# edlanglois/relearn

Measured on AMD Instinct MI355X. Metric: env-steps/sec (whole node), 64k-env CartPole TRPO, higher is better.
Workload: dtype f32; 1 GPU; CartPole(VisibleStepLimit 500) MLP-TRPO, 65536 envs total, T=128, policy 5-128-2, critic 5-128-1, CG 10, <=15 backtracks, 80 Adam critic steps per period; n_envs_total=65536, n_envs_per_gpu=65536, horizon=128, hidden=128, critic_steps=80, update_chains=policy and critic chains side by side on two streams, pipeline=none, parallelism=env-sharded x1 + no collective (one rank)

## Files before the change

### relearn_amd/csrc/abi_internal.hpp

```cpp
#pragma once
#include <cmath>
#include <cstdlib>
#include <cstring>
#include <memory>
#include <string>
#include <vector>

#include "../../include/rl_chacha.h"
#include "../../include/rl_detmath.h"
#include "engine.hpp"
#include "host/cbor.hpp"
#include "kernels.hpp"

extern thread_local std::string g_last_error_no_engine;

static inline void engine_settle(rl_engine *e) {
  if (e->pending.active && !e->pending.joined) {
    RL_HIP_CHECK(hipStreamWaitEvent(e->main_stream, e->ev_join, 0));
    e->pending.joined = true;
  }
}

template <typename F>
static inline int32_t guarded(rl_engine *eng, F &&f, bool settle = true) {
// ... 59 lines not shown
                    "rl_engine_set_kernel_variant(engine, 1) for these magnitudes (include/relearn_hip.h)");
}
static inline void range_discard(rl_traj *t) {
  try {
    range_check(t);
  } catch (const RlError &) {
  }
}

enum PassKind { RUN_INIT = PASS_INIT, RUN_EVAL = PASS_EVAL, RUN_JVP = PASS_JVP, RUN_DQN = PASS_DQN, RUN_PPO = PASS_PPO,
                RUN_CRITIC, RUN_KINDS };
struct SlabRows {
  uint32_t A, B;
};
struct PassRequest {
  PassRequest(PassKind k) : kind(k) {}
  PassKind kind;
  const float *tangent = nullptr;
  const int32_t *skip = nullptr;
  float clip_lo = 0.0f, clip_hi = 0.0f;
  bool forward_only = false;
  bool reduce = true;
  uint64_t B_total = 0;
};
SlabRows run_pass(const rl_mlp *mod, rl_traj *traj, const PassRequest &req);

extern "C" {
void engine_release_child(rl_engine *e);
void traj_plan(rl_traj *t, uint64_t B);
rl_traj *traj_alloc(rl_engine *e, uint64_t n_lanes, uint64_t horizon, uint32_t obs_dim, bool resizable);
void seq_ensure(rl_traj *t, const rl_mlp *mod, bool training);
void traj_ensure_pvec(rl_traj *t, uint64_t P);
rl_mlp *seq_exec(const rl_mlp *m);
}

struct SeqScope {
  rl_traj *t;
  uint32_t logical_D;
  rl_mlp *x;
  SeqScope(rl_traj *traj, const rl_mlp *m) : t(traj), logical_D(traj->d.D), x(nullptr) {
    RL_REQUIRE(m->in_dim == traj->d.D, "module input width does not match the trajectory");
    x = seq_exec(m);
    if (!m->lane_kernels()) t->d.D = 5;
  }
  ~SeqScope() { t->d.D = logical_D; }
  SeqScope(const SeqScope &) = delete;
// ... 3 lines not shown
```

### relearn_amd/csrc/abi_update.hip

```cpp
#include "abi_internal.hpp"

enum FusedLauncher { FUSED_NONE, FUSED_POLICY ,
                     FUSED_CRITIC  };
struct PassRow {
  bool backward, sums;
  FusedLauncher fused;
};
static const PassRow PASS_TABLE[RUN_KINDS] = {
     {true, true, FUSED_POLICY},
     {false, true, FUSED_POLICY},
     {true, false, FUSED_POLICY},
     {true, true, FUSED_NONE},
     {true, true, FUSED_POLICY},
     {true, true, FUSED_CRITIC},
};
static_assert(RUN_INIT == 0 && RUN_EVAL == 1 && RUN_JVP == 2 && RUN_DQN == 3 && RUN_PPO == 4 && RUN_CRITIC == 5 &&
                  RUN_KINDS == 6,
              "PASS_TABLE rows are in the order of PassKind");

static void seq_gradient_to_flat_order(const rl_mlp *mod, rl_traj *traj) {
  if (mod->exec == nullptr) return;
  launch_seq_unpad(mod, traj->vec, mod->x_tmp);
  RL_HIP_CHECK(hipMemcpyAsync(traj->vec, mod->x_tmp, mod->P * sizeof(float), hipMemcpyDeviceToDevice, traj->eng->stream));
}
// ... 20 lines not shown
      const float *tangent = req.tangent;
      if (mod->exec != nullptr) {
        launch_seq_pad(mod, mod->x_tan, req.tangent);
        tangent = mod->x_tan;
      }
      launch_gru_tangent(traj, sc.x, tangent, Bt, req.skip);
    } else {
      launch_gru_seq_forward(traj, sc.x, traj->seq.out, nullptr, row.backward ? seq_record(traj, sc.x) : nullptr,
                             req.skip);
      if (critic) launch_seq_critic_dvalues(traj, Bt);
      else launch_seq_policy_dlogits(traj, req.kind, Bt, req.clip_lo, req.clip_hi, req.skip);
    }
    if (grad) {
      launch_gru_backward(traj, sc.x, req.skip);
      seq_gradient_to_flat_order(mod, traj);
    }
    if (row.sums) launch_reduce(traj, P, false, true, 0, traj->nbB);
    allreduce();
    return SlabRows{0, traj->nbB};
  }
  bool fused = false;
  if (traj->eng->kernel_variant == 0) {
    if (row.fused == FUSED_POLICY)
      fused = launch_policy_v2(traj, mod, req.kind, req.tangent, Bt, req.skip, req.clip_lo, req.clip_hi);
    else if (row.fused == FUSED_CRITIC)
      fused = launch_critic_step_v2(traj, mod, Bt);
  }
  if (!fused) {
    if (critic) launch_critic_fwd(traj, mod, Bt);
    else launch_policy_pass(traj, mod, req.kind, req.tangent, Bt, req.skip, req.clip_lo, req.clip_hi);
    if (row.backward) launch_mlp_backward(traj, mod, req.skip);
  }
  const SlabRows rows = fused ? SlabRows{traj->last_rows, traj->last_rows} : SlabRows{traj->nbA, traj->nbB};
  if (req.reduce) {
    launch_reduce(traj, P, row.backward, row.sums, rows.A, rows.B);
    allreduce();
  }
  return rows;
}

extern "C" {

int32_t rl_trpo_config_default(rl_trpo_config *c) {
  return guarded(nullptr, [&] {
    RL_REQUIRE(c, "cfg is NULL");
    c->iterations = 10;
    c->max_backtracks = 15;
// ... 12 lines not shown
             "policy outputs do not match the action count of the env this trajectory was collected on");
  RL_REQUIRE(policy->out_dim > traj->max_action, "the trajectory holds an action index the policy has no output for");
  if (policy->out_dim > 2 && policy->kind != RL_MODULE_MLP)
    throw RlError(RL_ERR_UNSUPPORTED, "recurrent chains are built for two actions");
}

static inline void trpo_candidate(rl_mlp *policy, rl_traj *traj, const rl_trpo_config *cfg, uint64_t i, double ratio) {
  launch_ls_set_params(traj, policy, ratio);
  PassRequest eval(RUN_EVAL);
  eval.skip = &traj->trpo->ls_accepted;
  run_pass(policy, traj, eval);
  launch_ls_check(traj, (uint32_t)policy->P, b_total(traj), (int)i, ratio, cfg->max_policy_step_kl);
}

struct TrpoProgress {
  uint64_t next = 0;
  double ratio = 1.0;
};

static TrpoProgress trpo_update_head(rl_mlp *policy, rl_traj *traj, const rl_trpo_config *cfg) {
  uint32_t P = (uint32_t)policy->P;
  uint64_t Bt = b_total(traj);
  float reg = (float)cfg->hpv_reg_coeff;
  run_pass(policy, traj, RUN_INIT);
  launch_trpo_begin(traj, policy, Bt);
  PassRequest fvp(RUN_JVP);
  fvp.tangent = traj->cg_p;
  fvp.skip = &traj->trpo->cg_done;
  for (uint64_t it = 0; it < cfg->iterations; ++it) {
    run_pass(policy, traj, fvp);
    launch_cg_step(traj, P, reg, 1e-10f);
  }
  launch_cg_finish(traj, P);
  fvp.tangent = traj->cg_x;
  fvp.skip = nullptr;
  run_pass(policy, traj, fvp);
  launch_step_size(traj, policy, reg, cfg->max_policy_step_kl);
  TrpoProgress pr;
  for (; pr.next < cfg->max_backtracks && pr.next < 2; ++pr.next) {
    if (pr.next > 0) pr.ratio *= cfg->backtrack_ratio;
    trpo_candidate(policy, traj, cfg, pr.next, pr.ratio);
  }
  return pr;
}

static void trpo_update_tail(rl_mlp *policy, rl_traj *traj, const rl_trpo_config *cfg, TrpoProgress pr,
                             rl_trpo_stats *stats) {
// ... 44 lines not shown
}

int32_t rl_policy_gradient(rl_mlp *policy, rl_traj *traj, float *grad_out, float *loss_out, float *entropy_out) {
  return guarded(traj ? traj->eng : nullptr, [&] {
    check_policy(policy, traj);
    RL_REQUIRE(grad_out, "grad_out is NULL");
    uint32_t P = (uint32_t)policy->P;
    run_pass(policy, traj, RUN_INIT);
    std::vector<float> h(P + 4);
    d2h(traj->eng, h.data(), traj->vec, (P + 4) * sizeof(float));
    range_check(traj, 1u << RL_GUARD_POLICY);
    std::memcpy(grad_out, h.data(), P * sizeof(float));
    double inv_B = 1.0 / (double)b_total(traj);
    if (loss_out) *loss_out = (float)(-((double)h[P] * inv_B));
    if (entropy_out) *entropy_out = (float)((double)h[P + 1] * inv_B);
  });
}

int32_t rl_policy_fvp(rl_mlp *policy, rl_traj *traj, const float *v, float reg, float *out) {
  return guarded(traj ? traj->eng : nullptr, [&] {
    check_policy(policy, traj);
    RL_REQUIRE(v && out, "NULL argument");
    uint32_t P = (uint32_t)policy->P;
    run_pass(policy, traj, RUN_INIT);
    h2d(traj->eng, traj->cg_x, v, P * sizeof(float));
    PassRequest fvp(RUN_JVP);
    fvp.tangent = traj->cg_x;
    run_pass(policy, traj, fvp);
    std::vector<float> h(P);
    d2h(traj->eng, h.data(), traj->vec, P * sizeof(float));
    range_check(traj, 1u << RL_GUARD_POLICY);
    for (uint32_t i = 0; i < P; ++i) out[i] = h[i] + reg * v[i];
  });
}

int32_t rl_policy_loss_kl(rl_mlp *policy, rl_traj *traj, const float *params0, float *loss_out, float *kl_out) {
  return guarded(traj ? traj->eng : nullptr, [&] {
    check_policy(policy, traj);
    RL_REQUIRE(params0 && loss_out && kl_out, "NULL argument");
    rl_engine *e = traj->eng;
    uint32_t P = (uint32_t)policy->P;
    uint64_t Bt = b_total(traj);
    std::vector<float> cur(P);
    d2h(e, cur.data(), policy->d_params, P * sizeof(float));
    h2d(e, policy->d_params, params0, P * sizeof(float));
    wimg_invalidate(policy);
    run_pass(policy, traj, RUN_INIT);
// ... 521 lines not shown
```

### relearn_amd/csrc/bf16_tile.hpp

```cpp
#pragma once
#include <hip/hip_runtime.h>

#include <cstdint>
#include <type_traits>

#include "../../include/rl_detmath.h"

namespace bt {

typedef float f32x16 __attribute__((ext_vector_type(16)));
typedef float f32x2 __attribute__((ext_vector_type(2)));
typedef __bf16 bf16x8 __attribute__((ext_vector_type(8)));
typedef __bf16 bf16x2 __attribute__((ext_vector_type(2)));

constexpr int NT = 4;
constexpr int PAR_D = 5, PAR_H = 128;
constexpr uint32_t PAR_B1 = PAR_H * PAR_D, PAR_W2 = PAR_B1 + PAR_H;
__host__ __device__ constexpr uint32_t par_b2(int A) { return PAR_W2 + (uint32_t)(A * PAR_H); }
constexpr uint32_t SHARE_OLD = 5, SHARE_YOUNG = 3;

__device__ __forceinline__ void wave_lds_fence() {
  __builtin_amdgcn_fence(__ATOMIC_RELEASE, "wavefront");
  __builtin_amdgcn_wave_barrier();
  __builtin_amdgcn_fence(__ATOMIC_ACQUIRE, "wavefront");
// ... 33 lines not shown
  float a[4] = {row[0], row[1], row[2], row[3]};
#pragma unroll
  for (int c = 4; c < 16; ++c) a[c & 3] = a[c & 3] + row[c];
  return (a[0] + a[1]) + (a[2] + a[3]);
}
constexpr int YROW = 36;
__device__ __forceinline__ float row_sum16v(const float *row) {
  const float4 *v = reinterpret_cast<const float4 *>(row);
  const float4 q0 = v[0], q1 = v[1], q2 = v[2], q3 = v[3];
  const float a0 = ((q0.x + q1.x) + q2.x) + q3.x, a1 = ((q0.y + q1.y) + q2.y) + q3.y;
  const float a2 = ((q0.z + q1.z) + q2.z) + q3.z, a3 = ((q0.w + q1.w) + q2.w) + q3.w;
  return (a0 + a1) + (a2 + a3);
}

typedef __amdgpu_buffer_rsrc_t rsrc_t;
__device__ __forceinline__ rsrc_t make_rsrc(const void *p, uint32_t bytes) {
  return __builtin_amdgcn_make_buffer_rsrc(const_cast<void *>(p), 0, (int)bytes, 0x00020000);
}
__device__ __forceinline__ float buf_f32(rsrc_t r, uint32_t lane_off, uint32_t tile_off) {
  return __builtin_bit_cast(float, __builtin_amdgcn_raw_buffer_load_b32(r, (int)lane_off, (int)tile_off, 0));
}
__device__ __forceinline__ uint32_t buf_u8(rsrc_t r, uint32_t lane_off, uint32_t tile_off) {
  return (uint32_t)__builtin_amdgcn_raw_buffer_load_b8(r, (int)lane_off, (int)tile_off, 0);
}

union Frag {
  bf16x8 v;
  uint32_t u[4];
  uint64_t q[2];
  uint4 x;
};

constexpr float FWD_SCALE = 0x1p96f, FWD_UNSCALE = 0x1p-96f;

constexpr int WIMG_RAW = 5;
constexpr int WIMG_FRAG_WORDS = NT * 3 * 64 * 4;
constexpr int WIMG_WORDS = WIMG_FRAG_WORDS + NT * WIMG_RAW * 64;
__device__ __forceinline__ uint32_t wimg_half_index(int t, int lane, int h) {
  return (uint32_t)(((t * 3 + (h >> 3)) * 64 + lane) * 8 + (h & 7));
}
__device__ __forceinline__ uint32_t wimg_raw_index(int t, int lane, int c) {
  return (uint32_t)(WIMG_FRAG_WORDS + (t * WIMG_RAW + c) * 64 + lane);
}
__device__ __forceinline__ void wimg_store_param(uint32_t *__restrict__ img, uint32_t p, float w, int A) {
  constexpr int H = PAR_H, D = PAR_D;
  unsigned short *h16 = reinterpret_cast<unsigned short *>(img);
// ... 313 lines not shown
  for (int t = 0; t < NT; ++t) {
    WRaw r;
    wimg_load(wimg, t, lane, fw[t], r, A);
    if (guard) range_guard_img(r, lane >> 5, xmin, xmax, range_err + CHAIN, range_veto(range, CHAIN));
    fold(t, r);
  }
}

struct Dealing {
  uint32_t share, first, n_waves;
};
template <int WAVES, int CHANNELS = 1>
__device__ __forceinline__ Dealing deal_tiles(int wave, uint32_t share_old, uint32_t share_young) {
  constexpr int WALKERS = WAVES / CHANNELS, HALF = WALKERS / 2;
  const int w = CHANNELS == 1 ? wave : wave & (WALKERS - 1);
  const uint32_t per_wg = HALF * (share_old + share_young);
  Dealing d;
  d.share = w < HALF ? share_old : share_young;
  d.first = blockIdx.x * per_wg +
            (w < HALF ? (uint32_t)w * share_old : HALF * share_old + (uint32_t)(w - HALF) * share_young);
  d.n_waves = gridDim.x * per_wg;
  return d;
}
template <bool TWO_BUFFERS, typename L, typename T>
__device__ __forceinline__ void walk_tiles(const Dealing &deal, uint32_t n_full, uint32_t tail, L &load_tile, T &tile) {
  const Dealing d = deal;
  for (uint32_t vw = 0; vw < d.share; ++vw) {
    const uint32_t wave_id = d.first + vw;
    if (wave_id < n_full) {
      auto op_a = load_tile(wave_id), op_b = op_a;
      if (!TWO_BUFFERS) {
        for (uint32_t g = wave_id; g < n_full; g += d.n_waves) {
          const uint32_t g1 = g + d.n_waves;
          op_b = load_tile(g1 < n_full ? g1 : g);
          tile(std::false_type{}, op_a, g);
          op_a = op_b;
        }
      } else {
        for (uint32_t g = wave_id; g < n_full; g += 2 * d.n_waves) {
          const uint32_t g1 = g + d.n_waves, g2 = g1 + d.n_waves;
          op_b = load_tile(g1 < n_full ? g1 : g);
          tile(std::false_type{}, op_a, g);
          if (g1 >= n_full) break;
          op_a = load_tile(g2 < n_full ? g2 : g1);
          tile(std::false_type{}, op_b, g1);
        }
      }
    }
    if (tail != 0 && n_full % d.n_waves == wave_id) tile(std::true_type{}, load_tile(n_full), n_full);
  }
}

template <int W, typename LIN>
__device__ __forceinline__ float transpose_sum(float (&ysh)[W][32][YROW], int w, const float (&yp)[16], LIN lin, int n,
                                               int hf) {
#pragma unroll
  for (int r = 0; r < 16; ++r) ysh[w][(r & 3) + 8 * (r >> 2) + 4 * hf][n] = yp[r];
  wave_lds_fence();
  float part = row_sum16v(&ysh[w][n][hf * 16]);
  part = part + lin();
  float p0, p1;
  both_halves(part, p0, p1);
  return p0 + p1;
}
__device__ __forceinline__ float linear_half(const float (&lv)[3], float xa, float xb, float xc, int hf) {
  float lin = lv[0] * xa;
  lin = __builtin_fmaf(lv[1], xb, lin);
  return __builtin_fmaf(lv[2], hf == 0 ? xc : 1.0f, lin);
}
// ... 31 lines not shown
```

### relearn_amd/csrc/engine.hpp

```cpp
#pragma once

#include <hip/hip_runtime.h>

#include <cstdint>
#include <cstdio>
#include <stdexcept>
#include <string>
#include <vector>

#include "../../include/relearn_hip.h"
#include "dev_mem.hpp"

struct RlError : std::runtime_error {
  int32_t code;
  RlError(int32_t c, const std::string &m) : std::runtime_error(m), code(c) {}
};

#define RL_HIP_CHECK(expr)                                                                          \
  do {                                                                                              \
    hipError_t _e = (expr);                                                                         \
    if (_e != hipSuccess)                                                                           \
      throw RlError(RL_ERR_HIP, std::string(#expr) + ": " + hipGetErrorString(_e) + " (" __FILE__ ":" + \
                                    std::to_string(__LINE__) + ")");                                \
  } while (0)
// ... 258 lines not shown
struct OptState {
  float *s0, *s1, *s2;
};

struct rl_adam {
  rl_engine *eng;
  DevMem mem;
  rl_mlp *mod;
  rl_optimizer_config cfg;
  float *d_state[3] = {nullptr, nullptr, nullptr};
  uint64_t *d_step = nullptr;
  uint64_t host_step = 0;
  uint64_t error_epoch = 0;
};

struct rl_traj {
  rl_engine *eng;
  DevMem mem;
  TrajDev d;
  uint64_t B;
  float *lp0 = nullptr;
  float *dz = nullptr;
  uint32_t act_planes = 2;
  uint32_t n_actions = 0, max_action = 0;
  double *slabA = nullptr;
  double *slabB = nullptr;
  float *vec = nullptr;
  float *cg_x = nullptr, *cg_r = nullptr, *cg_p = nullptr, *prev_params = nullptr, *descent = nullptr;
  float *td = nullptr;
  float *losses = nullptr;
  TrpoStateDev *trpo = nullptr;
  uint32_t nbA = 0, nbB = 0, nbV2 = 0, nbC = 0, Pmax = 0, max_losses = 0;
  uint32_t last_rows = 0;
  double *aux_slabA = nullptr, *aux_slabB = nullptr;
  float *aux_vec = nullptr;
  uint32_t aux_last_rows = 0;
  bool range_valid = false, range_fixed = false;
  bool range_reset = false;
  uint32_t *h_range_err = nullptr;
  bool guard_next_policy = true, guard_next_critic = true;
  bool rtg_scan_valid = false;
  float rtg_gamma = 0.0f;
  const float *last_targets = nullptr;
  uint32_t bwd_chunk = 0;
  SeqDev seq;
  GenDev gen;
// ... 51 lines not shown
```

### relearn_amd/csrc/kernels.hpp

```cpp
#pragma once
#include <cstdlib>
#include <functional>
#define RL_SEQ_ACT_ARRAYS 9
#define RL_SEQ_DPRE_ARRAYS 6
#include "engine.hpp"

void launch_env_reset(rl_env *env);
void launch_env_observe(rl_env *env, float *d_obs);
void launch_env_step(rl_env *env);
void launch_rollout(rl_env *env, const rl_mlp *policy, rl_traj *traj);
void launch_values(rl_traj *traj, const rl_mlp *critic);
void launch_gae(rl_traj *traj, const rl_mlp *critic, float gamma, float lambda);
void launch_value_targets(rl_traj *traj, const rl_mlp *critic, float gamma);
void launch_mlp_forward_host_rows(rl_mlp *mlp, const float *d_in_soa, size_t rows, float *d_out_soa);
void launch_obs_range(rl_traj *traj);
inline void traj_ensure_range(rl_traj *traj) {
  if (traj->range_valid || traj->range_fixed) return;
  launch_obs_range(traj);
  traj->range_valid = true;
}
inline bool fused_5_128_fits(const rl_traj *t, const rl_mlp *m, uint32_t out_dim, bool offsets = true) {
  return m->kind == RL_MODULE_MLP && !m->general && t->d.D == 5 && m->hidden == 128 && m->out_dim == out_dim &&
         (!offsets || (uint64_t)(t->d.T + 1) * t->d.n * 5 < (1ull << 30));
}
// ... 21 lines not shown
  t->mem.ensure(t->seq.succ, 2 * B);
}

enum PolicyPassMode { PASS_INIT = 0, PASS_EVAL = 1, PASS_JVP = 2, PASS_DQN = 3, PASS_PPO = 4 };
void launch_policy_pass(rl_traj *traj, const rl_mlp *policy, int mode, const float *d_tangent, uint64_t B_total,
                        const int32_t *d_skip_flag, float clip_lo = 0.0f, float clip_hi = 0.0f);
void launch_critic_fwd(rl_traj *traj, const rl_mlp *critic, uint64_t B_total);
void launch_mlp_backward(rl_traj *traj, const rl_mlp *mlp, const int32_t *d_skip_flag);
void launch_reduce(rl_traj *traj, uint32_t P, bool useA, bool useB, uint32_t rowsA, uint32_t rowsB);

void launch_trpo_begin(rl_traj *traj, rl_mlp *policy, uint64_t B_total);
void launch_cg_step(rl_traj *traj, uint32_t P, float reg, float tol);
void launch_cg_finish(rl_traj *traj, uint32_t P);
void launch_step_size(rl_traj *traj, rl_mlp *policy, float reg, double max_kl);
void launch_ls_set_params(rl_traj *traj, rl_mlp *policy, double ratio);
void launch_ls_check(rl_traj *traj, uint32_t P, uint64_t B_total, int index, double ratio, double max_kl);
void launch_ls_finalize(rl_traj *traj, rl_mlp *policy, double max_kl, int accept_violation);
void launch_opt_step(rl_traj *traj, rl_adam *opt, int loss_slot, uint64_t B_total);
void launch_opt_step_vec(rl_adam *opt, const float *d_grad);
void launch_reduce_opt(rl_traj *traj, rl_adam *opt, uint32_t rowsA, uint32_t rowsB, int loss_slot, uint64_t B_total);

bool launch_critic_step_v2(rl_traj *traj, const rl_mlp *critic, uint64_t B_total);
bool launch_policy_v2(rl_traj *traj, const rl_mlp *policy, int mode, const float *d_tangent, uint64_t B_total,
                      const int32_t *d_skip_flag, float clip_lo = 0.0f, float clip_hi = 0.0f);

void launch_rollout_dqn(rl_env *env, const rl_mlp *qnet, const ReplayDev &rp, uint32_t T, uint64_t p_int,
                        int always_explore, uint8_t *d_flags, uint32_t *d_range = nullptr);
void launch_rollout_dqn_general(rl_env *env, const rl_mlp *qnet, rl_traj *ws, float *d_q, const ReplayDev &rp, uint32_t T,
                                uint64_t p_int, int always_explore, uint8_t *d_flags);
void launch_dqn_td_targets(rl_engine *eng, float *d_target, const uint8_t *d_flag, const float *d_q_next, uint32_t n,
                           float gamma);
struct AgentKey { uint32_t w[8]; };
void launch_dqn_sample(rl_engine *eng, hipStream_t stream, const ReplayDev &rp, const AgentKey &key, uint64_t *d_agent_pos,
                       uint32_t minibatch_steps, uint32_t max_eps, uint32_t *d_lane, uint32_t *d_start,
                       uint32_t *d_len, uint32_t *d_off, DqnCountsDev *d_counts, int sequential,
                       uint32_t n_batches = 1);
void launch_dqn_build_all(rl_engine *eng, const ReplayDev &rp, uint32_t n_batches, uint32_t widest_eps, uint32_t max_eps,
                          const uint32_t *d_lane, const uint32_t *d_start, const uint32_t *d_len, const uint32_t *d_off,
                          const DqnCountsDev *d_counts, float *d_obs, size_t obs_stride, uint8_t *d_action,
                          float *d_target, size_t step_stride, float gamma, uint8_t *d_flag);
void launch_replay_planes(rl_engine *eng, const ReplayDev &rp, int field, void *d_out);
bool launch_dqn_step_bf16(rl_traj *mb, const rl_mlp *qnet, uint64_t B_total, float gamma);
bool launch_dqn_step_pair(rl_traj *mb, const rl_mlp *qnet, uint64_t B_total);
void launch_dqn_build_minibatch(rl_engine *eng, const ReplayDev &rp, uint32_t n_eps, const uint32_t *d_lane,
                                const uint32_t *d_start, const uint32_t *d_len, const uint32_t *d_off,
                                float *d_obs, size_t out_plane, uint8_t *d_action, float *d_target, float gamma,
                                int one_step_td, const rl_mlp *qnet);
// ... 47 lines not shown
```

### relearn_amd/csrc/kernels_critic.hip

```cpp
#include <type_traits>

#include "bf16_tile.hpp"
#include "device_fns.hpp"
#include "kernels.hpp"

static_assert(bt::RANGE_WORDS == RL_RANGE_WORDS && bt::RANGE_ALLOC_WORDS == RL_RANGE_ALLOC_WORDS &&
                  bt::GUARD_POLICY == RL_GUARD_POLICY && bt::GUARD_CRITIC == RL_GUARD_CRITIC,
              "engine.hpp and bf16_tile.hpp describe the same range / veto words");

using bt::f32x16;
using bt::Frag;

constexpr int CRITIC_WAVES = 8;
constexpr int C_FLUSH = 64;

template <int CH>
__global__ void __launch_bounds__(CRITIC_WAVES * 64, 2)
    k_critic_step_mfma(TrajDev tr, const float *__restrict__ params, const uint32_t *__restrict__ wimg,
                       double *__restrict__ slabA, double *__restrict__ slabB, float two_over_B, uint32_t P,
                       uint32_t share_old, uint32_t share_young) {
  constexpr int D = 5, H = 128, NT = bt::NT;
  constexpr int IMG = H * 7 + 2;
  __shared__ __attribute__((aligned(16))) float Ysh[CRITIC_WAVES][32][bt::YROW];
  __shared__ double Acc[CRITIC_WAVES][IMG];
// ... 83 lines not shown
    const float y =
        0.5f * bt::transpose_sum(Ysh, wave, yp, [&] { return bt::linear_half(lv, op.xa, op.xb, op.xc, hf); }, n, hf) + b2;
    const float d = y - op.tgt;
    const bool mine = CH == 2 ? valid && op.act == (uint32_t)chan : valid;
    const float dy = mine ? d * two_over_B : 0.0f;
    if (mine) {
      loss32 = __builtin_fmaf(d, d, loss32);
      db2_32 = db2_32 + dy;
    }
    Frag ub[2];
    bt::piece_frags_mfma(dy, op.xa, op.xb, op.xc, hf, selb, ub);
    bt::backward(ga, ub, dm);
    bt::wave_lds_fence();
    if (++since_flush == C_FLUSH) {
      since_flush = 0;
      bt::flush(dm, acc64, 7, n, hf, !flushed);
      flushed = true;
      loss64 += (double)loss32;
      db2_64 += (double)db2_32;
      loss32 = db2_32 = 0.0f;
    }
  };

  bt::walk_tiles<true>(deal, n_full, tail, load_tile, tile);
  if (since_flush != 0 || !flushed) {
    bt::flush(dm, acc64, 7, n, hf, !flushed);
    loss64 += (double)loss32;
    db2_64 += (double)db2_32;
  }
  const double l = bt::owner_sum(loss64, hf), bsum = bt::owner_sum(db2_64, hf);
  if (lane == 0) {
    acc64[H * 7] = bsum;
    acc64[H * 7 + 1] = l;
  }
  __syncthreads();
  for (uint32_t p = threadIdx.x; p <= P; p += CRITIC_WAVES * 64) {
    auto tot = [&](int src) { return bt::image_sum<CRITIC_WAVES>(Acc, src); };
    auto totc = [&](int c, int src) { return bt::image_sum<CRITIC_WAVES / 2>(Acc + 4 * c, src); };
    double s;
    if (p >= bt::par_b2(CH)) {
      s = p == P ? tot(H * 7 + 1) : CH == 2 ? totc((int)(p - bt::par_b2(CH)), H * 7) : tot(H * 7);
    } else if (CH == 2) {
      s = bt::grad_entry<2>(p, params, [&](int c, int j, int k) { return totc(c, j * 7 + k); },
                            [&](int c, int j) { return (double)W2[c * H + j]; });
    } else {
      s = bt::grad_entry<1>(p, params, [&](int, int j, int k) { return tot(j * 7 + k); },
                            [&](int, int j) { return (double)W2[j]; });
// ... 36 lines not shown
```

### relearn_amd/csrc/kernels_mfma.hip

```cpp
#include <type_traits>

#include "bf16_tile.hpp"
#include "device_fns.hpp"
#include "kernels.hpp"
#include "policy_fast.hpp"

constexpr int V2_WAVES = 8;

constexpr int PB_FLUSH = 16;

template <int MODE, int WAVES, bool FW_LDS = false>
__global__ void __launch_bounds__(WAVES * 64)
    k_policy_bf16(TrajDev tr, const float *__restrict__ params, const uint32_t *__restrict__ wimg,
                  const float *__restrict__ tangent, float *__restrict__ lp0, double *__restrict__ slabA,
                  double *__restrict__ slabB, float inv_B, uint32_t P, const int32_t *__restrict__ skip, float clip_lo,
                  float clip_hi, uint32_t share_old, uint32_t share_young) {
  using bt::Frag;
  constexpr int D = 5, H = 128, NT = bt::NT, A = 2;
  constexpr bool BWD = MODE != PASS_EVAL;
  constexpr bool JVP = MODE == PASS_JVP;
  constexpr int IW = 7;
  constexpr int PIMG_M = H * IW + 5;
  __shared__ __attribute__((aligned(16))) float Ysh[JVP ? 1 : WAVES][32][bt::YROW];
  __shared__ double Acc[WAVES][BWD ? PIMG_M : 4];
  __shared__ uint4 Fz[JVP ? bt::L2_KS : 1][64];
  __shared__ uint4 Fw[FW_LDS ? NT * 3 : 1][64];
  if (skip != nullptr && *skip != 0) return;

  const int lane = threadIdx.x & 63;
  const int wave = __builtin_amdgcn_readfirstlane((int)(threadIdx.x >> 6));
  const int n = lane & 31, hf = lane >> 5;
  const float *__restrict__ W1 = params, *__restrict__ b1 = W1 + bt::PAR_B1, *__restrict__ W2 = params + bt::PAR_W2,
                           *__restrict__ b2 = params + bt::par_b2(A);
  const size_t B = (size_t)tr.T * tr.n;
  const size_t plane = (size_t)(tr.T + 1) * tr.n;
  double *acc64 = Acc[wave];
  bool flushed = false;

  Frag fw[NT][3];
  float w2d[NT];
  float lvd[3] = {0.0f, 0.0f, 0.0f};
  float tb2d = 0.0f;
  bt::load_weights<bt::GUARD_POLICY>(wimg, wave, lane, 2, tr.range, tr.range_err, fw, [&](int t, const bt::WRaw &r) {
    if (FW_LDS && wave == t) {
#pragma unroll
      for (int i = 0; i < 3; ++i) Fw[t * 3 + i][lane] = fw[t][i].x;
    }
    const float wd = r.w2[0] - r.w2[1];
    if (!JVP) {
      lvd[0] = __builtin_fmaf(wd, r.wa, lvd[0]);
      lvd[1] = __builtin_fmaf(wd, r.wb, lvd[1]);
      lvd[2] = __builtin_fmaf(wd, r.wc, lvd[2]);
    }
    w2d[t] = bt::FWD_UNSCALE * wd;
  });
  if (JVP) {
    const float *__restrict__ V1 = tangent, *__restrict__ vb1 = V1 + bt::PAR_B1, *__restrict__ V2 = tangent + bt::PAR_W2;
    bt::l2_build(Fz, (int)threadIdx.x, WAVES * 64, [&](int j, int k) {
      const float wd = W2[j] - W2[H + j], t2d = V2[j] - V2[H + j];
      const float w = k < D ? W1[j * D + k] : b1[j], v = k < D ? V1[j * D + k] : vb1[j];
      return __builtin_fmaf(t2d, w, wd * v);
    });
  }
  if (JVP || FW_LDS) __syncthreads();
  if (JVP) {
    const float *__restrict__ vb2 = tangent + bt::par_b2(A);
    tb2d = vb2[0] - vb2[1];
  } else {
#pragma unroll
    for (int q = 0; q < 3; ++q) lvd[q] = bt::half_sum(lvd[q]);
  }
  const float b2d = b2[0] - b2[1];
  Frag selb[2], idb[2];
  if (BWD) bt::sel_frags(lane, selb);
  if (JVP) bt::ident_frags(lane, idb);
  bt::f32x16 dm[NT];
#pragma unroll
  for (int t = 0; t < NT; ++t) dm[t] = (bt::f32x16){0, 0, 0, 0, 0, 0, 0, 0, 0, 0, 0, 0, 0, 0, 0, 0};
  double sum0 = 0.0, sum1 = 0.0, sum2 = 0.0, db2_0 = 0.0, db2_1 = 0.0;
  float s0f = 0.0f, s1f = 0.0f, s2f = 0.0f, d0f = 0.0f, d1f = 0.0f;
  auto fold = [&]() {
    sum0 += (double)s0f;
    sum1 += (double)s1f;
    sum2 += (double)s2f;
    db2_0 += (double)d0f;
    db2_1 += (double)d1f;
    s0f = s1f = s2f = d0f = d1f = 0.0f;
  };
  bt::wave_lds_fence();

  const uint32_t B32 = (uint32_t)B, plane32 = (uint32_t)plane;
  const uint32_t n_full = B32 / 32u, tail = B32 & 31u;
  if (WAVES != 8) share_old = share_young = 1u;
  const bt::Dealing deal = bt::deal_tiles<WAVES>(wave, share_old, share_young);
  const bt::rsrc_t obs_r = bt::make_rsrc(tr.obs, (uint32_t)D * plane32 * 4u), lp0_r = bt::make_rsrc(lp0, 2u * B32 * 4u);
  const bt::rsrc_t adv_r = bt::make_rsrc(tr.adv, B32 * 4u), act_r = bt::make_rsrc(tr.action, B32);
  const uint32_t off_a = ((uint32_t)(2 * hf) * plane32 + (uint32_t)n) * 4u, off_b = off_a + plane32 * 4u;
  const uint32_t off_c = (4u * plane32 + (uint32_t)n) * 4u, off_s = (uint32_t)n * 4u, off_s1 = off_s + B32 * 4u;
  int since_flush = 0;
  struct TileOp {
    float xa, xb, xc, l0, l1, adv;
    int act;
  };
  auto load_tile = [&](uint32_t g) {
    TileOp o;
    const uint32_t soff = g * 128u;
    o.xa = bt::buf_f32(obs_r, off_a, soff);
    o.xb = bt::buf_f32(obs_r, off_b, soff);
    o.xc = bt::buf_f32(obs_r, off_c, soff);
    o.l0 = o.l1 = o.adv = 0.0f;
    o.act = 0;
    if (MODE != PASS_INIT) {
      o.l0 = bt::buf_f32(lp0_r, off_s, soff);
      o.l1 = bt::buf_f32(lp0_r, off_s1, soff);
    }
    if (!JVP) {
      o.adv = bt::buf_f32(adv_r, off_s, soff);
      o.act = (int)bt::buf_u8(act_r, (uint32_t)n, g * 32u);
    }
    return o;
  };
  auto tile = [&](auto ragged, TileOp op_in, uint32_t g) {
    constexpr bool RAGGED = decltype(ragged)::value;
    struct {
      float xa, xb, xc, l0, l1, adv;
      int act;
      bool valid;
    } op;
    op.valid = RAGGED ? (uint32_t)n < tail : true;
    op.xa = op.valid ? op_in.xa : 0.0f;
    op.xb = op.valid ? op_in.xb : 0.0f;
    op.xc = op.valid ? op_in.xc : 0.0f;
    op.l0 = op.valid ? op_in.l0 : 0.0f;
    op.l1 = op.valid ? op_in.l1 : 0.0f;
    op.adv = op.valid ? op_in.adv : 0.0f;
    op.act = op.valid ? op_in.act : 0;
    const size_t sidx = (size_t)g * 32 + n;
    Frag fa[3];
    bt::input_frags(op.xa, op.xb, op.xc, op.valid, hf, fa);
    Frag ga[NT][2];
    float y0[16];
#pragma unroll
    for (int r = 0; r < 16; ++r) y0[r] = 0.0f;
    bt::f32x16 q = {0, 0, 0, 0, 0, 0, 0, 0, 0, 0, 0, 0, 0, 0, 0, 0};
    auto fwd = [&](int t) {
      if (FW_LDS) {
        Frag f[3];
#pragma unroll
        for (int i = 0; i < 3; ++i) f[i].x = Fw[t * 3 + i][lane];
        return bt::layer1(fa, f);
      }
      return bt::layer1(fa, fw[t]);
    };
    bt::f32x16 c = fwd(0);
#pragma unroll
    for (int t = 0; t < NT; ++t) {
      bt::f32x16 cn = c;
      if (t + 1 < NT) cn = fwd(t + 1);
      if (!JVP) {
#pragma unroll
        for (int r = 0; r < 16; ++r) y0[r] = __builtin_fmaf(__builtin_fabsf(c[r]), w2d[t], y0[r]);
      }
      if (BWD) bt::mask_tile(c, ga[t]);
      if (JVP) q = bt::masked_sum_tile(ga[t], idb, Fz, t, lane, q);
      c = cn;
    }
    float s0;
    if (JVP) {
      float p0, p1;
      bt::both_halves(bt::l2_dot(q, op.xa, op.xb, hf == 0 ? op.xc : 1.0f), p0, p1);
      s0 = p0 + p1;
    } else {
      s0 = 0.5f * bt::transpose_sum(
                      Ysh, JVP ? 0 : wave, y0, [&] { return bt::linear_half(lvd, op.xa, op.xb, op.xc, hf); }, n, hf);
      bt::wave_lds_fence();
    }
    float dz0 = 0.0f, dz1 = 0.0f;
    if (JVP) {
      const float delta = s0 + tb2d;
      const SoftPair old = soft_pair(op.l0 - op.l1);
      dz0 = op.valid ? (old.p[0] * old.p[1]) * delta * inv_B : 0.0f;
      dz1 = -dz0;
    } else {
      const float adv = op.adv;
      const int act = op.act;
      const SoftPair sp = soft_pair(s0 + b2d);
      const float(&lp)[2] = sp.lp;
      if (MODE == PASS_PPO) {
        const float l0a = act == 0 ? op.l0 : op.l1;
        const float lpa = act == 0 ? lp[0] : lp[1];
        const float ratio = fast_expf(lpa - l0a);
        const float clipped = ratio < clip_lo ? clip_lo : (ratio > clip_hi ? clip_hi : ratio);
        const float u1 = ratio * adv, u2 = clipped * adv;
        const bool inside = ratio >= clip_lo && ratio <= clip_hi;
        const float gr = u1 < u2 ? adv : (u1 > u2 ? (inside ? adv : 0.0f) : (inside ? adv : 0.5f * adv));
        const float cc = -(gr * ratio) * inv_B;
        dz0 = op.valid ? cc * ((act == 0 ? 1.0f : 0.0f) - sp.p[0]) : 0.0f;
        dz1 = op.valid ? cc * ((act == 1 ? 1.0f : 0.0f) - sp.p[1]) : 0.0f;
        if (op.valid) s0f = s0f + (u1 < u2 ? u1 : u2);
      } else if (MODE == PASS_INIT) {
        if (op.valid && hf == 0) {
          lp0[sidx] = lp[0];
          lp0[B + sidx] = lp[1];
        }
        const float lpa = act == 0 ? lp[0] : lp[1];
        const float ratio = fast_expf(lpa - lpa);
        const float cc = -(ratio * adv) * inv_B;
        const float pa0 = sp.p[0], pa1 = sp.p[1];
        dz0 = op.valid ? cc * ((act == 0 ? 1.0f : 0.0f) - pa0) : 0.0f;
        dz1 = op.valid ? cc * ((act == 1 ? 1.0f : 0.0f) - pa1) : 0.0f;
        const float cl0 = lp[0] < -3.402823466e+38f ? -3.402823466e+38f : lp[0];
        const float cl1 = lp[1] < -3.402823466e+38f ? -3.402823466e+38f : lp[1];
        float ent = cl0 * pa0;
        ent += cl1 * pa1;
        if (op.valid) {
          s0f = __builtin_fmaf(ratio, adv, s0f);
          s1f = s1f - ent;
          s2f = __builtin_fmaf(lpa, adv, s2f);
        }
      } else {
        const float l00 = op.l0, l01 = op.l1;
        const float lpa = act == 0 ? lp[0] : lp[1];
        const float l0a = act == 0 ? l00 : l01;
        const float ratio = fast_expf(lpa - l0a);
        float rel0 = l00 - lp[0], rel1 = l01 - lp[1];
        if (rel0 < -3.402823466e+38f) rel0 = -3.402823466e+38f;
// ... 4 lines not shown
        if (op.valid) {
          s0f = __builtin_fmaf(ratio, adv, s0f);
          s1f = s1f + kl;
        }
      }
    }
    if (BWD) {
      d0f = d0f + dz0;
      d1f = d1f + dz1;
      Frag ub[2];
      bt::piece_frags_mfma(0.5f * (dz0 - dz1), op.xa, op.xb, op.xc, hf, selb, ub);
      bt::backward(ga, ub, dm);
      if (++since_flush == PB_FLUSH) {
        since_flush = 0;
        bt::flush(dm, acc64, IW, n, hf, !flushed);
        flushed = true;
        fold();
      }
    } else if (++since_flush == PB_FLUSH) {
      since_flush = 0;
      fold();
    }
  };
  bt::walk_tiles<!JVP>(deal, n_full, tail, load_tile, tile);
  if (BWD && (since_flush != 0 || !flushed)) bt::flush(dm, acc64, IW, n, hf, !flushed);
  fold();
  const double r0 = bt::owner_sum(sum0, hf), r1 = bt::owner_sum(sum1, hf);
  const double r2 = bt::owner_sum(db2_0, hf), r3 = bt::owner_sum(db2_1, hf);
  const double r4 = MODE == PASS_INIT ? bt::owner_sum(sum2, hf) : 0.0;
  constexpr int TAIL = BWD ? H * IW : 0;
  if (lane == 0) {
    if (BWD) {
      acc64[TAIL + 0] = r2;
      acc64[TAIL + 1] = r3;
      acc64[TAIL + 2] = r0;
      acc64[TAIL + 3] = r1;
      if (MODE == PASS_INIT) acc64[TAIL + 4] = r4;
    } else {
      acc64[0] = r0;
      acc64[1] = r1;
    }
  }
  __syncthreads();
  auto tot = [&](int src) { return bt::image_sum<WAVES>(Acc, src); };
  if (BWD) {
    for (uint32_t p = threadIdx.x; p < P; p += WAVES * 64) {
      double s;
      if (p < bt::par_b2(A)) {
        s = bt::grad_entry<1>(p, params, [&](int, int j, int k) { return tot(j * IW + k); },
                              [&](int, int j) { return (double)W2[j] - (double)W2[H + j]; });
        if (p >= bt::PAR_W2 + H) s = -s;
      } else {
        s = tot(TAIL + (int)(p - bt::par_b2(A)));
      }
      slabA[(size_t)blockIdx.x * P + p] = s;
    }
  }
  if (threadIdx.x < 4) {
    double v = 0.0;
    if (BWD) {
      if (!JVP && threadIdx.x < 2) v = tot(TAIL + 2 + threadIdx.x);
      if (MODE == PASS_INIT && threadIdx.x == 2) v = tot(TAIL + 4);
    } else if (threadIdx.x < 2) {
      v = tot(threadIdx.x);
    }
    slabB[(size_t)blockIdx.x * 4 + threadIdx.x] = v;
  }
}

bool launch_policy_v2(rl_traj *traj, const rl_mlp *policy, int mode, const float *d_tangent, uint64_t B_total,
                      const int32_t *d_skip, float clip_lo, float clip_hi) {
  if (policy->general) return launch_gen_mfma(traj, policy, mode, d_tangent, B_total, d_skip, clip_lo, clip_hi);
  if (!fused_5_128_fits(traj, policy, 2)) return false;
  if (mode == PASS_DQN) return false;
  traj_ensure_range(traj);
  const uint32_t *wimg = wimg_ensure(policy);
  ProfScope ps(traj->eng, mode == PASS_JVP ? RL_K_POLICY_FVP : RL_K_POLICY_FUSED);
  float inv_B = 1.0f / (float)B_total;
  traj->nbV2 = fused_grid(traj, V2_WAVES);
  traj->last_rows = traj->nbV2;
  dim3 g(traj->nbV2), b(V2_WAVES * 64);
  hipStream_t s = traj->eng->stream;
  uint32_t P = (uint32_t)policy->P;
  const TrajDev d = fused_traj_dev(traj, traj->guard_next_policy);
#define BLAUNCH(MM)                                                                                                  \
  hipLaunchKernelGGL((k_policy_bf16<MM, V2_WAVES>), g, b, 0, s, d, policy->d_params, wimg, d_tangent, traj->lp0,       \
                     traj->slabA, traj->slabB, inv_B, P, d_skip, clip_lo, clip_hi, bt::SHARE_OLD, bt::SHARE_YOUNG)
  if (mode == PASS_INIT) BLAUNCH(PASS_INIT);
  else if (mode == PASS_JVP) BLAUNCH(PASS_JVP);
  else if (mode == PASS_PPO) BLAUNCH(PASS_PPO);
  else {
    constexpr int EVAL_WAVES = 16;
    hipLaunchKernelGGL((k_policy_bf16<PASS_EVAL, EVAL_WAVES, true>), g, dim3(EVAL_WAVES * 64), 0, s, d,
                       policy->d_params, wimg, d_tangent, traj->lp0, traj->slabA, traj->slabB, inv_B, P, d_skip, clip_lo,
                       clip_hi, 1u, 1u);
  }
#undef BLAUNCH
  return true;
}
```

Before: 483.4 million env-steps/s.

## Cache ReLU masks and softmax weights from gradient pass for Fisher-vector passes

The TRPO gradient (INIT) pass now stores a compact bit-packed ReLU-derivative mask per sample plus the old-policy p0*p1 weight. Each of the conjugate-gradient Fisher-vector passes reads these instead of recomputing the layer-1 forward matmul and softmax, skipping weight loading and input fragments in JVP mode. walk_tiles is also unified to always use the two-buffer schedule. The cost is extra memory traffic, 8 bytes of mask and 4 bytes of weight per sample written once and read every CG iteration, plus an epoch check that throws if the cache is stale.

```diff
diff --git a/relearn_amd/csrc/abi_internal.hpp b/relearn_amd/csrc/abi_internal.hpp
--- a/relearn_amd/csrc/abi_internal.hpp
+++ b/relearn_amd/csrc/abi_internal.hpp
@@ -105,6 +105,7 @@
   bool forward_only = false;
   bool reduce = true;
   uint64_t B_total = 0;
+  bool keep = false;
 };
 SlabRows run_pass(const rl_mlp *mod, rl_traj *traj, const PassRequest &req);
 
diff --git a/relearn_amd/csrc/abi_update.hip b/relearn_amd/csrc/abi_update.hip
--- a/relearn_amd/csrc/abi_update.hip
+++ b/relearn_amd/csrc/abi_update.hip
@@ -66,7 +66,7 @@
   bool fused = false;
   if (traj->eng->kernel_variant == 0) {
     if (row.fused == FUSED_POLICY)
-      fused = launch_policy_v2(traj, mod, req.kind, req.tangent, Bt, req.skip, req.clip_lo, req.clip_hi);
+      fused = launch_policy_v2(traj, mod, req.kind, req.tangent, Bt, req.skip, req.clip_lo, req.clip_hi, req.keep);
     else if (row.fused == FUSED_CRITIC)
       fused = launch_critic_step_v2(traj, mod, Bt);
   }
@@ -125,7 +125,9 @@
   uint32_t P = (uint32_t)policy->P;
   uint64_t Bt = b_total(traj);
   float reg = (float)cfg->hpv_reg_coeff;
-  run_pass(policy, traj, RUN_INIT);
+  PassRequest init(RUN_INIT);
+  init.keep = true;
+  run_pass(policy, traj, init);
   launch_trpo_begin(traj, policy, Bt);
   PassRequest fvp(RUN_JVP);
   fvp.tangent = traj->cg_p;
@@ -216,7 +218,9 @@
     check_policy(policy, traj);
     RL_REQUIRE(v && out, "NULL argument");
     uint32_t P = (uint32_t)policy->P;
-    run_pass(policy, traj, RUN_INIT);
+    PassRequest init(RUN_INIT);
+    init.keep = true;
+    run_pass(policy, traj, init);
     h2d(traj->eng, traj->cg_x, v, P * sizeof(float));
     PassRequest fvp(RUN_JVP);
     fvp.tangent = traj->cg_x;
diff --git a/relearn_amd/csrc/bf16_tile.hpp b/relearn_amd/csrc/bf16_tile.hpp
--- a/relearn_amd/csrc/bf16_tile.hpp
+++ b/relearn_amd/csrc/bf16_tile.hpp
@@ -79,6 +79,13 @@
 }
 __device__ __forceinline__ uint32_t buf_u8(rsrc_t r, uint32_t lane_off, uint32_t tile_off) {
   return (uint32_t)__builtin_amdgcn_raw_buffer_load_b8(r, (int)lane_off, (int)tile_off, 0);
+}
+typedef uint32_t u32x2 __attribute__((ext_vector_type(2)));
+__device__ __forceinline__ u32x2 buf_u32x2(rsrc_t r, uint32_t lane_off, uint32_t tile_off) {
+  return __builtin_bit_cast(u32x2, __builtin_amdgcn_raw_buffer_load_b64(r, (int)lane_off, (int)tile_off, 0));
+}
+__device__ __forceinline__ void buf_store_u32x2(u32x2 v, rsrc_t r, uint32_t lane_off, uint32_t tile_off) {
+  __builtin_amdgcn_raw_buffer_store_b64(v, r, (int)lane_off, (int)tile_off, 0);
 }
 
 union Frag {
@@ -438,29 +445,20 @@
   d.n_waves = gridDim.x * per_wg;
   return d;
 }
-template <bool TWO_BUFFERS, typename L, typename T>
+template <typename L, typename T>
 __device__ __forceinline__ void walk_tiles(const Dealing &deal, uint32_t n_full, uint32_t tail, L &load_tile, T &tile) {
   const Dealing d = deal;
   for (uint32_t vw = 0; vw < d.share; ++vw) {
     const uint32_t wave_id = d.first + vw;
     if (wave_id < n_full) {
       auto op_a = load_tile(wave_id), op_b = op_a;
-      if (!TWO_BUFFERS) {
-        for (uint32_t g = wave_id; g < n_full; g += d.n_waves) {
-          const uint32_t g1 = g + d.n_waves;
-          op_b = load_tile(g1 < n_full ? g1 : g);
-          tile(std::false_type{}, op_a, g);
-          op_a = op_b;
-        }
-      } else {
-        for (uint32_t g = wave_id; g < n_full; g += 2 * d.n_waves) {
-          const uint32_t g1 = g + d.n_waves, g2 = g1 + d.n_waves;
-          op_b = load_tile(g1 < n_full ? g1 : g);
-          tile(std::false_type{}, op_a, g);
-          if (g1 >= n_full) break;
-          op_a = load_tile(g2 < n_full ? g2 : g1);
-          tile(std::false_type{}, op_b, g1);
-        }
+      for (uint32_t g = wave_id; g < n_full; g += 2 * d.n_waves) {
+        const uint32_t g1 = g + d.n_waves, g2 = g1 + d.n_waves;
+        op_b = load_tile(g1 < n_full ? g1 : g);
+        tile(std::false_type{}, op_a, g);
+        if (g1 >= n_full) break;
+        op_a = load_tile(g2 < n_full ? g2 : g1);
+        tile(std::false_type{}, op_b, g1);
       }
     }
     if (tail != 0 && n_full % d.n_waves == wave_id) tile(std::true_type{}, load_tile(n_full), n_full);
diff --git a/relearn_amd/csrc/engine.hpp b/relearn_amd/csrc/engine.hpp
--- a/relearn_amd/csrc/engine.hpp
+++ b/relearn_amd/csrc/engine.hpp
@@ -304,6 +304,10 @@
   float *lp0 = nullptr;
   float *dz = nullptr;
   uint32_t act_planes = 2;
+  uint32_t *kept_mask = nullptr;
+  float *kept_w = nullptr;
+  uint64_t kept_epoch = 0, kept_samples = 0;
+  const rl_mlp *kept_policy = nullptr;
   uint32_t n_actions = 0, max_action = 0;
   double *slabA = nullptr;
   double *slabB = nullptr;
diff --git a/relearn_amd/csrc/kernels.hpp b/relearn_amd/csrc/kernels.hpp
--- a/relearn_amd/csrc/kernels.hpp
+++ b/relearn_amd/csrc/kernels.hpp
@@ -67,7 +67,7 @@
 
 bool launch_critic_step_v2(rl_traj *traj, const rl_mlp *critic, uint64_t B_total);
 bool launch_policy_v2(rl_traj *traj, const rl_mlp *policy, int mode, const float *d_tangent, uint64_t B_total,
-                      const int32_t *d_skip_flag, float clip_lo = 0.0f, float clip_hi = 0.0f);
+                      const int32_t *d_skip_flag, float clip_lo = 0.0f, float clip_hi = 0.0f, bool keep = false);
 
 void launch_rollout_dqn(rl_env *env, const rl_mlp *qnet, const ReplayDev &rp, uint32_t T, uint64_t p_int,
                         int always_explore, uint8_t *d_flags, uint32_t *d_range = nullptr);
diff --git a/relearn_amd/csrc/kernels_critic.hip b/relearn_amd/csrc/kernels_critic.hip
--- a/relearn_amd/csrc/kernels_critic.hip
+++ b/relearn_amd/csrc/kernels_critic.hip
@@ -129,7 +129,7 @@
     }
   };
 
-  bt::walk_tiles<true>(deal, n_full, tail, load_tile, tile);
+  bt::walk_tiles(deal, n_full, tail, load_tile, tile);
   if (since_flush != 0 || !flushed) {
     bt::flush(dm, acc64, 7, n, hf, !flushed);
     loss64 += (double)loss32;
diff --git a/relearn_amd/csrc/kernels_mfma.hip b/relearn_amd/csrc/kernels_mfma.hip
--- a/relearn_amd/csrc/kernels_mfma.hip
+++ b/relearn_amd/csrc/kernels_mfma.hip
@@ -3,18 +3,21 @@
 #include "bf16_tile.hpp"
 #include "device_fns.hpp"
 #include "kernels.hpp"
+#include "mask_plane.hpp"
 #include "policy_fast.hpp"
 
 constexpr int V2_WAVES = 8;
 
 constexpr int PB_FLUSH = 16;
 
-template <int MODE, int WAVES, bool FW_LDS = false>
+template <int MODE, int WAVES, bool FW_LDS = false, bool KEEP = false>
 __global__ void __launch_bounds__(WAVES * 64)
     k_policy_bf16(TrajDev tr, const float *__restrict__ params, const uint32_t *__restrict__ wimg,
                   const float *__restrict__ tangent, float *__restrict__ lp0, double *__restrict__ slabA,
                   double *__restrict__ slabB, float inv_B, uint32_t P, const int32_t *__restrict__ skip, float clip_lo,
-                  float clip_hi, uint32_t share_old, uint32_t share_young) {
+                  float clip_hi, uint32_t share_old, uint32_t share_young, uint32_t *__restrict__ kept_mask,
+                  float *__restrict__ kept_w) {
+  static_assert(!KEEP || MODE == PASS_INIT, "only the gradient pass keeps");
   using bt::Frag;
   constexpr int D = 5, H = 128, NT = bt::NT, A = 2;
   constexpr bool BWD = MODE != PASS_EVAL;
@@ -41,19 +44,18 @@
   float w2d[NT];
   float lvd[3] = {0.0f, 0.0f, 0.0f};
   float tb2d = 0.0f;
-  bt::load_weights<bt::GUARD_POLICY>(wimg, wave, lane, 2, tr.range, tr.range_err, fw, [&](int t, const bt::WRaw &r) {
+  auto fold_raw = [&](int t, const bt::WRaw &r) {
     if (FW_LDS && wave == t) {
 #pragma unroll
       for (int i = 0; i < 3; ++i) Fw[t * 3 + i][lane] = fw[t][i].x;
     }
     const float wd = r.w2[0] - r.w2[1];
-    if (!JVP) {
-      lvd[0] = __builtin_fmaf(wd, r.wa, lvd[0]);
-      lvd[1] = __builtin_fmaf(wd, r.wb, lvd[1]);
-      lvd[2] = __builtin_fmaf(wd, r.wc, lvd[2]);
-    }
+    lvd[0] = __builtin_fmaf(wd, r.wa, lvd[0]);
+    lvd[1] = __builtin_fmaf(wd, r.wb, lvd[1]);
+    lvd[2] = __builtin_fmaf(wd, r.wc, lvd[2]);
     w2d[t] = bt::FWD_UNSCALE * wd;
-  });
+  };
+  if (!JVP) bt::load_weights<bt::GUARD_POLICY>(wimg, wave, lane, 2, tr.range, tr.range_err, fw, fold_raw);
   if (JVP) {
     const float *__restrict__ V1 = tangent, *__restrict__ vb1 = V1 + bt::PAR_B1, *__restrict__ V2 = tangent + bt::PAR_W2;
     bt::l2_build(Fz, (int)threadIdx.x, WAVES * 64, [&](int j, int k) {
@@ -97,10 +99,15 @@
   const bt::rsrc_t adv_r = bt::make_rsrc(tr.adv, B32 * 4u), act_r = bt::make_rsrc(tr.action, B32);
   const uint32_t off_a = ((uint32_t)(2 * hf) * plane32 + (uint32_t)n) * 4u, off_b = off_a + plane32 * 4u;
   const uint32_t off_c = (4u * plane32 + (uint32_t)n) * 4u, off_s = (uint32_t)n * 4u, off_s1 = off_s + B32 * 4u;
+  const uint32_t n_tiles32 = (B32 + 31u) / 32u;
+  const bt::rsrc_t km_r = bt::make_rsrc(kept_mask, n_tiles32 * mp::TILE_BYTES), kw_r = bt::make_rsrc(kept_w, B32 * 4u);
+  const uint32_t off_m = mp::lane_offset(lane);
   int since_flush = 0;
   struct TileOp {
     float xa, xb, xc, l0, l1, adv;
     int act;
+    uint32_t m[mp::WORDS];
+    float w;
   };
   auto load_tile = [&](uint32_t g) {
     TileOp o;
@@ -108,9 +115,15 @@
     o.xa = bt::buf_f32(obs_r, off_a, soff);
     o.xb = bt::buf_f32(obs_r, off_b, soff);
     o.xc = bt::buf_f32(obs_r, off_c, soff);
-    o.l0 = o.l1 = o.adv = 0.0f;
+    o.l0 = o.l1 = o.adv = o.w = 0.0f;
     o.act = 0;
-    if (MODE != PASS_INIT) {
+    o.m[0] = o.m[1] = 0u;
+    if (JVP) {
+      const bt::u32x2 mw = bt::buf_u32x2(km_r, off_m, mp::tile_offset(g));
+      o.m[0] = mw[0];
+      o.m[1] = mw[1];
+      o.w = bt::buf_f32(kw_r, off_s, soff);
+    } else if (MODE != PASS_INIT) {
       o.l0 = bt::buf_f32(lp0_r, off_s, soff);
       o.l1 = bt::buf_f32(lp0_r, off_s1, soff);
     }
@@ -135,9 +148,10 @@
     op.l1 = op.valid ? op_in.l1 : 0.0f;
     op.adv = op.valid ? op_in.adv : 0.0f;
     op.act = op.valid ? op_in.act : 0;
+    const float kw_in = op.valid ? op_in.w : 0.0f;
     const size_t sidx = (size_t)g * 32 + n;
     Frag fa[3];
-    bt::input_frags(op.xa, op.xb, op.xc, op.valid, hf, fa);
+    if (!JVP) bt::input_frags(op.xa, op.xb, op.xc, op.valid, hf, fa);
     Frag ga[NT][2];
     float y0[16];
 #pragma unroll
@@ -152,18 +166,32 @@
       }
       return bt::layer1(fa, fw[t]);
     };
-    bt::f32x16 c = fwd(0);
-#pragma unroll
-    for (int t = 0; t < NT; ++t) {
-      bt::f32x16 cn = c;
-      if (t + 1 < NT) cn = fwd(t + 1);
-      if (!JVP) {
+    if (JVP) {
+#pragma unroll
+      for (int t = 0; t < NT; ++t) {
+#pragma unroll
+        for (int s = 0; s < 2; ++s)
+#pragma unroll
+          for (int i = 0; i < 4; ++i) ga[t][s].u[i] = mp::decode_pair(op_in.m, mp::pair_index(t, s, i));
+        q = bt::masked_sum_tile(ga[t], idb, Fz, t, lane, q);
+      }
+    } else {
+      uint32_t grp[NT];
+      bt::f32x16 c = fwd(0);
+#pragma unroll
+      for (int t = 0; t < NT; ++t) {
+        bt::f32x16 cn = c;
+        if (t + 1 < NT) cn = fwd(t + 1);
 #pragma unroll
         for (int r = 0; r < 16; ++r) y0[r] = __builtin_fmaf(__builtin_fabsf(c[r]), w2d[t], y0[r]);
-      }
-      if (BWD) bt::mask_tile(c, ga[t]);
-      if (JVP) q = bt::masked_sum_tile(ga[t], idb, Fz, t, lane, q);
-      c = cn;
+        if (BWD) bt::mask_tile(c, ga[t]);
+        if (KEEP) grp[t] = mp::encode_group([&](int k) { return ga[t][k >> 2].u[k & 3]; });
+        c = cn;
+      }
+      if (KEEP) {
+        const bt::u32x2 mw = {mp::encode_word(grp[0], grp[1]), mp::encode_word(grp[2], grp[3])};
+        bt::buf_store_u32x2(mw, km_r, off_m, mp::tile_offset(g));
+      }
     }
     float s0;
     if (JVP) {
@@ -178,8 +206,7 @@
     float dz0 = 0.0f, dz1 = 0.0f;
     if (JVP) {
       const float delta = s0 + tb2d;
-      const SoftPair old = soft_pair(op.l0 - op.l1);
-      dz0 = op.valid ? (old.p[0] * old.p[1]) * delta * inv_B : 0.0f;
+      dz0 = op.valid ? kw_in * delta * inv_B : 0.0f;
       dz1 = -dz0;
     } else {
       const float adv = op.adv;
@@ -202,6 +229,10 @@
         if (op.valid && hf == 0) {
           lp0[sidx] = lp[0];
           lp0[B + sidx] = lp[1];
+          if (KEEP) {
+            const SoftPair old = soft_pair(lp[0] - lp[1]);
+            kept_w[sidx] = old.p[0] * old.p[1];
+          }
         }
         const float lpa = act == 0 ? lp[0] : lp[1];
         const float ratio = fast_expf(lpa - lpa);
@@ -252,7 +283,7 @@
       fold();
     }
   };
-  bt::walk_tiles<!JVP>(deal, n_full, tail, load_tile, tile);
+  bt::walk_tiles(deal, n_full, tail, load_tile, tile);
   if (BWD && (since_flush != 0 || !flushed)) bt::flush(dm, acc64, IW, n, hf, !flushed);
   fold();
   const double r0 = bt::owner_sum(sum0, hf), r1 = bt::owner_sum(sum1, hf);
@@ -298,11 +329,27 @@
   }
 }
 
+static void traj_ensure_kept_planes(rl_traj *t) {
+  const uint64_t samples = (uint64_t)t->d.n * t->d.T;
+  t->mem.ensure(t->kept_mask, mp::plane_words(samples));
+  t->mem.ensure(t->kept_w, samples);
+}
+
 bool launch_policy_v2(rl_traj *traj, const rl_mlp *policy, int mode, const float *d_tangent, uint64_t B_total,
-                      const int32_t *d_skip, float clip_lo, float clip_hi) {
+                      const int32_t *d_skip, float clip_lo, float clip_hi, bool keep) {
   if (policy->general) return launch_gen_mfma(traj, policy, mode, d_tangent, B_total, d_skip, clip_lo, clip_hi);
   if (!fused_5_128_fits(traj, policy, 2)) return false;
   if (mode == PASS_DQN) return false;
+  keep = keep && mode == PASS_INIT;
+  if (keep) {
+    traj->kept_epoch = 0;
+    traj_ensure_kept_planes(traj);
+  }
+  if (mode == PASS_JVP && !(traj->kept_epoch == traj->eng->call_epoch && traj->kept_policy == policy &&
+                            traj->kept_samples == traj->B && traj->kept_mask != nullptr && traj->kept_w != nullptr))
+    throw RlError(RL_ERR_UNSUPPORTED,
+                  "internal error: a Fisher-vector pass without a keeping gradient pass of the same policy and trajectory "
+                  "before it in the same call (its relu' masks would be stale)");
   traj_ensure_range(traj);
   const uint32_t *wimg = wimg_ensure(policy);
   ProfScope ps(traj->eng, mode == PASS_JVP ? RL_K_POLICY_FVP : RL_K_POLICY_FUSED);
@@ -315,15 +362,25 @@
   const TrajDev d = fused_traj_dev(traj, traj->guard_next_policy);
 #define BLAUNCH(MM)                                                                                                  \
   hipLaunchKernelGGL((k_policy_bf16<MM, V2_WAVES>), g, b, 0, s, d, policy->d_params, wimg, d_tangent, traj->lp0,       \
-                     traj->slabA, traj->slabB, inv_B, P, d_skip, clip_lo, clip_hi, bt::SHARE_OLD, bt::SHARE_YOUNG)
-  if (mode == PASS_INIT) BLAUNCH(PASS_INIT);
-  else if (mode == PASS_JVP) BLAUNCH(PASS_JVP);
+                     traj->slabA, traj->slabB, inv_B, P, d_skip, clip_lo, clip_hi, bt::SHARE_OLD, bt::SHARE_YOUNG,      \
+                     traj->kept_mask, traj->kept_w)
+  if (keep) {
+    hipLaunchKernelGGL((k_policy_bf16<PASS_INIT, V2_WAVES, false, true>), g, b, 0, s, d, policy->d_params, wimg,
+                       d_tangent, traj->lp0, traj->slabA, traj->slabB, inv_B, P, d_skip, clip_lo, clip_hi, bt::SHARE_OLD,
+                       bt::SHARE_YOUNG, traj->kept_mask, traj->kept_w);
+    traj->kept_epoch = traj->eng->call_epoch;
+    traj->kept_policy = policy;
+    traj->kept_samples = traj->B;
+  } else if (mode == PASS_INIT) {
+    traj->kept_epoch = 0;
+    BLAUNCH(PASS_INIT);
+  } else if (mode == PASS_JVP) BLAUNCH(PASS_JVP);
   else if (mode == PASS_PPO) BLAUNCH(PASS_PPO);
   else {
     constexpr int EVAL_WAVES = 16;
     hipLaunchKernelGGL((k_policy_bf16<PASS_EVAL, EVAL_WAVES, true>), g, dim3(EVAL_WAVES * 64), 0, s, d,
                        policy->d_params, wimg, d_tangent, traj->lp0, traj->slabA, traj->slabB, inv_B, P, d_skip, clip_lo,
-                       clip_hi, 1u, 1u);
+                       clip_hi, 1u, 1u, nullptr, nullptr);
   }
 #undef BLAUNCH
   return true;
diff --git a/relearn_amd/csrc/mask_plane.hpp b/relearn_amd/csrc/mask_plane.hpp
--- /dev/null
+++ b/relearn_amd/csrc/mask_plane.hpp
@@ -0,0 +1,49 @@
+#pragma once
+#include <cstdint>
+
+#if defined(__HIPCC__)
+#include <hip/hip_runtime.h>
+#define RL_MP_FN __host__ __device__ __forceinline__
+#else
+#define RL_MP_FN inline
+#endif
+
+namespace mp {
+
+constexpr int PAIRS = 32;
+constexpr int WORDS = 2;
+constexpr uint32_t LANE_BYTES = 8u;
+constexpr uint32_t TILE_BYTES = 512u;
+constexpr uint32_t ONE_PAIR = 0x3F803F80u;
+
+RL_MP_FN constexpr int pair_index(int t, int s, int i) { return 8 * t + 4 * s + i; }
+RL_MP_FN constexpr int pair_word(int q) { return q >> 4; }
+RL_MP_FN constexpr int pair_pos(int q) { return q & 15; }
+RL_MP_FN constexpr uint32_t tile_offset(uint32_t g) { return g * TILE_BYTES; }
+RL_MP_FN constexpr uint32_t lane_offset(int lane) { return (uint32_t)lane * LANE_BYTES; }
+RL_MP_FN constexpr uint64_t plane_words(uint64_t samples) { return (samples + 31) / 32 * (TILE_BYTES / 4); }
+
+template <typename F>
+RL_MP_FN uint32_t encode_group(F pair) {
+  uint32_t acc = pair(0) & (0x00010001u << 7);
+#if defined(__HIPCC__)
+#pragma unroll
+#endif
+  for (int k = 1; k < 7; ++k) {
+    const uint32_t m = 0x00010001u << (7 + k);
+    acc = (acc & ~m) | (pair(k) & m);
+  }
+  const uint32_t m = 0x00010001u << 14;
+  return (acc & ~m) | ((pair(7) << 1) & m);
+}
+RL_MP_FN uint32_t encode_word(uint32_t group_even, uint32_t group_odd) { return (group_even >> 7) | (group_odd << 1); }
+
+RL_MP_FN uint32_t mul24(uint32_t a, uint32_t b) { return (a & 0xFFFFFFu) * (b & 0xFFFFFFu); }
+RL_MP_FN uint32_t decode_source(uint32_t w, int h) { return h == 0 ? w : w >> 8; }
+RL_MP_FN uint32_t decode_pos(uint32_t src, int r7) { return mul24(src & (0x00010001u << r7), 0x3F80u >> r7); }
+RL_MP_FN uint32_t decode_pair(const uint32_t (&w)[WORDS], int q) {
+  const int r = pair_pos(q);
+  return decode_pos(decode_source(w[pair_word(q)], r >> 3), r & 7);
+}
+
+}
```

Result: faster. 495.8 million env-steps/s (median of 6 runs) (+2.6%).
